# Bismarrck/tensoralloy

Measured on AMD Instinct MI355X. Metric: atom-steps/sec (energy+forces), 4000-atom Ni rcut=6.5 A, higher is better.
Workload: dtype f64

## Files before the change

### tensoralloy_amd/csrc/ta_api.hip

```cpp
#include <hip/hip_runtime.h>

#include <algorithm>
#include <chrono>
#include <climits>
#include <cmath>
#include <cstdio>
#include <cstdlib>
#include <cstring>
#include <stdexcept>
#include <string>
#include <vector>

#include "ta_device.h"
#include "ta_internal.h"
#include "ta_md.h"
#include "ta_neb.h"
#include "ta_relax.h"

namespace ta {
size_t mlp_scratch_doubles(const MlpDev &mlp);
void launch_mlp_impl(const MlpDev &mlp, int activation, int ndim, const int32_t *atoms, int n_atoms,
                     const DeviceBatch &b, const Options &opt, double *scratch, hipStream_t s,
                     MlpLaunchInfo *info = nullptr);
size_t mlp_all_scratch_doubles(const MlpDev *mlps_host, int nel, const int32_t *elem_start);
// ... 716 lines not shown
      if (h->nl_zero.ptr != before || h->nl_zero_atoms != (int64_t)N || h->nl_zero_bins != n_bins) h->nl_zero_clean = false;
      h->nl_zero_atoms = (int64_t)N;
      h->nl_zero_bins = n_bins;
    }
    h->nl_rev_done = false;
    for (int attempt = 0; attempt < 2 && !h->nl_sorted; ++attempt) {
      const size_t capacity = std::min(std::min(h->pair_i.cap, h->pair_j.cap), h->pair_shift.cap / 3);
      h->pair_rev.ensure(capacity);
      const size_t guess = (hp.n_atoms == (int64_t)N && hp.n_pairs > 0) ? (size_t)hp.n_pairs + (size_t)hp.n_pairs / 4 + 4096
                                                                         : capacity;
      const size_t rev_cover = std::min(std::min(capacity, guess), (size_t)INT32_MAX);
      NlWork w = nl_work(h);
      nl_build((int)N, n_bins, nel, h->r_list, h->db.pos, h->db.species, h->db.frame_of_atom, h->d_grids, w,
               h->nl_zero.ptr, h->nl_zero_clean, (long long)std::min<size_t>(capacity, (size_t)INT32_MAX), h->pair_start.ptr,
               kernel_writes_host ? starts : nullptr, h->pair_i.ptr, h->pair_j.ptr, h->pair_shift.ptr,
               h->pair_rev.ptr, (long long)rev_cover, s);
      HIP_CHECK(hipGetLastError());
      h->nl_zero_clean = false;
      if (!kernel_writes_host)
        staged_copy(reinterpret_cast<double *>(starts), reinterpret_cast<const double *>(h->pair_start.ptr),
                    (N + 2) / 2, true, h->opt, s);
      staged_copy(reinterpret_cast<double *>(stats), reinterpret_cast<const double *>(h->nl_zero.ptr), 8, true, h->opt, s);
      wait_stream(s, h->opt);
      h->nl_zero_clean = N > 0;
      if (si[3] != 0) break;
      if (stats[4] > (unsigned long long)INT32_MAX) throw std::runtime_error("batch too large for 32-bit pair indices");
      if (stats[4] <= capacity) {
        h->nl_sorted = true;
        h->nl_rev_done = stats[4] <= rev_cover;
        if (h->nl_rev_done && si[6] != 0)
          throw std::runtime_error("neighbour list is not symmetric (reverse pair missing)");
      } else {
        h->pair_i.ensure((size_t)stats[4]);
        h->pair_j.ensure((size_t)stats[4]);
        h->pair_shift.ensure(3 * (size_t)stats[4]);
      }
    }
    if (h->nl_sorted) h->nl_stats_ptr = h->nl_zero.ptr;
  }
  if (!h->nl_sorted) {
    h->nl_bin_count.ensure((size_t)n_bins + 1);
    h->nl_bin_cursor.ensure((size_t)n_bins + 1);
    h->nl_counts.ensure(N * (nel + 1) + 1);
    h->nl_stats.ensure(8);
    NlWork w = nl_work(h);
    nl_count((int)N, n_bins, nel, h->r_list, h->db.pos, h->db.species, h->db.frame_of_atom, h->d_grids, w,
             h->pair_start.ptr, s);
    HIP_CHECK(hipGetLastError());
    HIP_CHECK(hipMemcpyAsync(stats, h->nl_stats.ptr, 8 * sizeof(unsigned long long), hipMemcpyDeviceToHost, s));
    HIP_CHECK(hipMemcpyAsync(starts, h->pair_start.ptr, (N + 1) * sizeof(int32_t), hipMemcpyDeviceToHost, s));
    HIP_CHECK(hipStreamSynchronize(s));
    if (stats[4] > (unsigned long long)INT32_MAX || si[4] < 0 || (unsigned long long)si[4] != stats[4])
      throw std::runtime_error("batch too large for 32-bit pair indices");
    h->nl_stats_ptr = h->nl_stats.ptr;
  }
  hp.n_atoms = (int64_t)N;
  hp.n_pairs = (int64_t)stats[4];
  hp.n_triples = (int64_t)stats[0];
  hp.nnl_max = si[2];
  hp.pair_start.assign(starts, starts + N + 1);
  hp.seg_start.clear();
  hp.pair_i.clear();
  hp.pair_j.clear();
  hp.pair_shift.clear();
  hp.pair_rev.clear();
  h->pairs_on_device = true;
}

void fill_pairs_on_device(ta_context *h) {
  using namespace ta;
  if (h->nl_sorted) {
    nl_reverse_sorted(h->hp.n_pairs, h->n_elements, h->db.species, h->seg_start.ptr, h->pair_i.ptr,
                      h->pair_j.ptr, h->pair_shift.ptr, h->pair_rev.ptr, h->nl_stats_ptr, h->stream);
  } else {
    NlWork w = nl_work(h);
    nl_fill((int)h->hp.n_atoms, h->hp.n_pairs, h->n_elements, h->r_list, h->db.pos, h->db.species,
            h->db.frame_of_atom, h->d_grids, w, h->pair_i.ptr, h->pair_j.ptr, h->pair_shift.ptr,
            h->pair_rev.ptr, h->stream);
  }
  HIP_CHECK(hipGetLastError());
}

#ifdef TA_PHASE_STAMPS
static void dump_stamps(ta_context *h) {
  const std::string &path = h->opt.phase_stamps_out;
  if (path.empty() || !h->db.stamps || h->db.n_blk <= 0) return;
  const size_t n = (size_t)2 * h->db.n_blk * ta::kStampSlots;
  std::vector<unsigned long long> v(n);
  (void)hipStreamSynchronize(h->stream);
  (void)hipMemcpy(v.data(), h->db.stamps, n * sizeof(unsigned long long), hipMemcpyDeviceToHost);
  FILE *fp = std::fopen(path.c_str(), "w");
  if (!fp) return;
  for (int k = 0; k < 2; ++k)
    for (int b = 0; b < h->db.n_blk; ++b) {
      std::fprintf(fp, "%d %d", k, b);
      for (int q = 0; q < ta::kStampSlots; ++q)
        std::fprintf(fp, " %llu", v[((size_t)k * h->db.n_blk + b) * ta::kStampSlots + q]);
      std::fprintf(fp, "\n");
    }
  std::fclose(fp);
}
#endif

void launch_head(ta_context *h, const ta::DeviceBatch &db, hipStream_t s) {
  if (h->td)
    ta::launch_td_all(h->td_dev, h->td_nets, h->n_elements, h->td_K, h->td_act, h->activation,
                      h->td_sommerfeld ? 1 : 0, h->sf.ndim, db, h->opt.mlp_da_global, h->td_T.ptr, h->td_u.ptr, h->td_s.ptr,
                      h->mlp_scratch.ptr, s, &h->last_mlp_launch);
  else
    ta::launch_mlp_all(h->mlp_dev, h->mlp, h->n_elements, h->activation, h->sf.ndim, db, h->opt, h->mlp_scratch.ptr,
                       s, &h->last_mlp_launch);
}

void forward_v2_launches(ta_context *h, bool tri) {
  using namespace ta;
  bool unread = tri && h->db.job_word_own && h->db.job_count_own && h->db.job_count;
  for (const ChunkPlan &cp : h->chunks_v2) unread = unread && v2_backward_takes_triangles(h->sf, cp.ch, cp.ng, cp.nz);
  bool geometry = true;
  size_t left = h->chunks_v2.size();
  for (const ChunkPlan &cp : h->chunks_v2) {
    --left;
    launch_g4_forward_v2(h->sf, cp.ch, cp.ng, cp.nz, geometry, left == 0, unread, h->db, h->opt, h->stream);
    geometry = false;
  }
  h->full_jobs_valid = !unread;
}

void compute_impl(ta_context *h, uint32_t want, bool timed, double *slot_ms) {
  using namespace ta;
#ifdef TA_PHASE_STAMPS
  if (h->db.n_blk > 0) {
    h->stamp_buf.ensure((size_t)2 * h->db.n_blk * ta::kStampSlots + 8);
    h->db.stamps = h->stamp_buf.ptr;
    (void)hipMemsetAsync(h->db.stamps, 0, (size_t)2 * h->db.n_blk * ta::kStampSlots * sizeof(unsigned long long),
                         h->stream);
  }
#endif
  h->db.rec4 = nullptr;
  h->db.own_sums = 0;
  const DeviceBatch &db = h->db;
  hipStream_t s = h->stream;
  const bool need_forces = (want & (TA_WANT_FORCES | TA_WANT_VIRIAL)) != 0;
  auto begin = [&](int slot) {
    if (timed) HIP_CHECK(hipEventRecord(h->ev[2 * slot], s));
  };
  auto end = [&](int slot) {
    if (timed) HIP_CHECK(hipEventRecord(h->ev[2 * slot + 1], s));
  };
  bool used[TA_N_KERNEL_SLOTS] = {false};

  const bool has_mlp = h->kind == TA_MODEL_SF_MLP || h->kind == TA_MODEL_GRAP_MLP;
  if ((want & TA_WANT_REUSE_DESCRIPTORS) && has_mlp && h->descriptors_valid && !need_forces) {
    begin(TA_K_MLP);
    launch_head(h, db, s);
    end(TA_K_MLP);
    used[TA_K_MLP] = true;
  } else if (h->kind == TA_MODEL_SF_MLP) {
    h->db.rec4 = (h->sf.angular && h->use_v2 && !h->opt.full_records) ? h->db.rec : nullptr;
    if (!h->use_v2) {
      begin(TA_K_PAIR_GEOMETRY);
      launch_pair_geometry(h->sf, db, s);
      end(TA_K_PAIR_GEOMETRY);
      used[TA_K_PAIR_GEOMETRY] = true;
    }
    h->sf.ang_scale = h->use_v2 ? 1.0 : 0.5;
    const bool tri_cells = (h->relax_cell_on || h->md_baro_on) ? h->tri_cells_wide_ok : h->tri_cells_ok;
    const bool tri = h->use_v2 && h->triangles && tri_cells && h->n_elements == 1 && need_forces;
    h->db.job_word_own = (tri && h->db.job_count) ? h->job_word_own.ptr : nullptr;
    h->db.job_count_own = (tri && h->db.job_count) ? h->job_count_own.ptr : nullptr;
    h->last_bwd_variant = 0;
    const bool reduce_in_forward = h->sf.angular && h->use_v2;
    if (h->sf.angular) {
      begin(TA_K_G4_FORWARD);
      if (h->use_v2)
        forward_v2_launches(h, tri);
      else
        for (const ChunkPlan &cp : h->chunks) launch_g4_forward(h->sf, cp.ch, cp.nb, cp.ng, cp.nz, db, s);
      end(TA_K_G4_FORWARD);
      used[TA_K_G4_FORWARD] = true;
    }
    if (!reduce_in_forward) {
      begin(TA_K_DESCRIPTOR_REDUCE);
      launch_descriptor_reduce(h->sf, db, s);
      end(TA_K_DESCRIPTOR_REDUCE);
      used[TA_K_DESCRIPTOR_REDUCE] = true;
    }
    begin(TA_K_MLP);
    launch_head(h, db, s);
    end(TA_K_MLP);
    used[TA_K_MLP] = true;
    if (need_forces) {
      begin(TA_K_BACKWARD);
      if (h->sf.angular) {
        bool first = true;
        if (h->use_v2)
          for (const ChunkPlan &cp : h->chunks_v2) {
            h->last_bwd_variant |= launch_backward_v2(h->sf, cp.ch, cp.ng, cp.nz, first, tri, db, h->opt, s);
            first = false;
          }
        else
          for (const ChunkPlan &cp : h->chunks) {
            launch_backward(h->sf, cp.ch, cp.nb, cp.ng, cp.nz, first, false, db, s);
            first = false;
          }
      } else {
        AngChunk dummy;
        std::memset(&dummy, 0, sizeof(dummy));
        launch_backward(h->sf, dummy, 1, 1, 1, true, true, db, s);
      }
      end(TA_K_BACKWARD);
      used[TA_K_BACKWARD] = true;
      begin(TA_K_FORCE_GATHER);
      launch_force_gather(h->sf, db, h->opt.gather_w, s);
      end(TA_K_FORCE_GATHER);
      used[TA_K_FORCE_GATHER] = true;
    }
  } else if (h->kind == TA_MODEL_GRAP_MLP) {
    const bool net_exact = ta::grap_uses_filter_net(h->grap) && !ta::grap_filter_table_knots(h->grap);
// ... 3056 lines not shown
```

### tensoralloy_amd/csrc/ta_mlp.hip

```cpp
#include <hip/hip_runtime.h>

#include <algorithm>
#include <cstdlib>
#include <map>
#include <mutex>
#include <stdexcept>

#include "ta_device.h"
#include "ta_mlp_tile.h"

namespace ta {
namespace {

constexpr int kMlpThreads = 256;

template <int THREADS>
__global__ __launch_bounds__(THREADS) void mlp_kernel(MlpDev mlp, int act, int ndim,
                                                          const int32_t *atoms, int n_atoms,
                                                          const double *G, double *dEdG,
                                                          double *eatom, double *scratch, int stride) {
  extern __shared__ double lds[];
  double *buf0 = lds, *buf1 = lds + kMlpRows * stride;
  const int a0 = blockIdx.x * kMlpRows;
  const int nrows = min(kMlpRows, n_atoms - a0);
  double *da = scratch ? scratch + (size_t)blockIdx.x * mlp.n_layers * kMlpRows * stride
                       : lds + 2 * kMlpRows * stride;
  for (int idx = threadIdx.x; idx < kMlpRows * ndim; idx += THREADS) {
    const int row = idx / ndim, k = idx - row * ndim;
    buf0[row * stride + k] = row < nrows ? G[(size_t)atoms[a0 + row] * ndim + k] : 0.0;
  }
  __syncthreads();
  mlp_tile<16>(
      mlp, act, ndim, nrows, buf0, buf1, stride, da,
      [&](int row, double y) { eatom[atoms[a0 + row]] = y; },
      [&](int row, int k, double d) { dEdG[(size_t)atoms[a0 + row] * ndim + k] = d; });
}

struct MlpTiles {
  int32_t tile_start[kMaxElements + 1];
  int32_t elem_start[kMaxElements + 1];
  int nel;
};

template <int THREADS>
__global__ __launch_bounds__(THREADS) void mlp_all_kernel(const MlpDev *__restrict__ mlps, MlpTiles tiles, int act,
                                                              int ndim, const int32_t *atoms,
                                                              const double *G, double *dEdG,
                                                              double *eatom, double *scratch,
                                                              int stride, int tile_doubles) {
  extern __shared__ double lds[];
  double *buf0 = lds, *buf1 = lds + kMlpRows * stride;
  int e = 0;
  while (e + 1 < tiles.nel && (int)blockIdx.x >= tiles.tile_start[e + 1]) ++e;
  const MlpDev &mlp = mlps[e];
  const int32_t *el_atoms = atoms + tiles.elem_start[e];
  const int n_atoms = tiles.elem_start[e + 1] - tiles.elem_start[e];
  const int a0 = ((int)blockIdx.x - tiles.tile_start[e]) * kMlpRows;
  const int nrows = min(kMlpRows, n_atoms - a0);
  double *da = scratch ? scratch + (size_t)blockIdx.x * tile_doubles : lds + 2 * kMlpRows * stride;
  for (int idx = threadIdx.x; idx < kMlpRows * ndim; idx += THREADS) {
    const int row = idx / ndim, k = idx - row * ndim;
    buf0[row * stride + k] = row < nrows ? G[(size_t)el_atoms[a0 + row] * ndim + k] : 0.0;
  }
  __syncthreads();
  mlp_tile<16>(
      mlp, act, ndim, nrows, buf0, buf1, stride, da,
      [&](int row, double y) { eatom[el_atoms[a0 + row]] = y; },
      [&](int row, int k, double d) { dEdG[(size_t)el_atoms[a0 + row] * ndim + k] = d; });
}

constexpr int kWaveNT = 4;
constexpr int kWaveThreads = 512;
constexpr int kWaveMaxHidden = 3;

constexpr int kWaveStride = 80;
__host__ __device__ inline int wave_stride(int x) { return (x % 32 == 0) ? x + 16 : x; }

struct WaveLds {
  const double *w[kWaveMaxHidden], *wt[kWaveMaxHidden], *b[kWaveMaxHidden];
  int swt0;
  const double *wout;
  double bout;
};

__host__ __device__ inline size_t wave_lds_doubles(const MlpDev &mlp, int lh) {
  size_t n = 0;
  for (int l = 0; l < lh; ++l) {
    const MlpLayerDev &ly = mlp.layer[l];
    n += (size_t)ly.kp * kWaveStride + (size_t)ly.np * (l == 0 ? wave_stride(ly.kp) : kWaveStride) + ly.np;
  }
  return n + mlp.layer[lh].kp;
}

__device__ __forceinline__ void wave_copy_rows(double *dst, int stride, const double *__restrict__ src, int rows,
                                               int cols) {
  const int n = rows * cols;
  for (int base = 0; base < n; base += 8 * kWaveThreads) {
    double v[8];
#pragma unroll
    for (int u = 0; u < 8; ++u) {
      const int idx = base + u * kWaveThreads + (int)threadIdx.x;
      v[u] = idx < n ? src[idx] : 0.0;
    }
#pragma unroll
    for (int u = 0; u < 8; ++u) {
      const int idx = base + u * kWaveThreads + (int)threadIdx.x;
      if (idx < n) {
        const int row = idx / cols;
        dst[row * stride + (idx - row * cols)] = v[u];
      }
    }
  }
}

template <int LH>
__device__ __forceinline__ void wave_stage(const MlpDev &mlp, double *lds, WaveLds &L) {
  double *p = lds;
#pragma unroll
// ... 148 lines not shown
      if (t < ntp) {
#pragma unroll
        for (int r = 0; r < 4; ++r) dh[l - 1][t][r] *= acc[t][r];
      }
  }
  {
    const MlpLayerDev &ly = mlp.layer[0];
    const int nt0 = ly.np / 16, swt = L.swt0;
    for (int j0 = 0; j0 < ndim; j0 += 16) {
      mlp_f64x4 acc = {0.0, 0.0, 0.0, 0.0};
      const double *wcol = L.wt[0] + kq * swt + j0 + m;
#pragma unroll
      for (int nt = 0; nt < kWaveNT; ++nt) {
        if (nt >= nt0) continue;
        double a[4];
#pragma unroll
        for (int r = 0; r < 4; ++r) a[r] = wcol[(16 * nt + 4 * r) * swt];
#pragma unroll
        for (int r = 0; r < 4; ++r) acc = __builtin_amdgcn_mfma_f64_16x16x4f64(a[r], dh[0][nt][r], acc, 0, 0, 0);
      }
#pragma unroll
      for (int r = 0; r < 4; ++r) {
        const int j = j0 + kq + 4 * r;
        if (valid && j < ndim) {
          double d = acc[r];
          if (mlp.xlo) {
            const double den = mlp.xhi[j] - mlp.xlo[j];
            d = (den != 0.0) ? -d / den : 0.0;
          }
          dEdG[(size_t)atom * ndim + j] = d;
        }
      }
    }
  }
}

template <int LH>
__global__ __launch_bounds__(kWaveThreads) void mlp_wave_kernel(MlpDev mlp, int act, int ndim, const int32_t *atoms,
                                                                int n_atoms, const double *G, double *dEdG,
                                                                double *eatom) {
  extern __shared__ double lds[];
  WaveLds L;
  wave_stage<LH>(mlp, lds, L);
  __syncthreads();
  const int ntiles = (n_atoms + kMlpRows - 1) / kMlpRows, nw = kWaveThreads / 64;
  for (int tile = (int)blockIdx.x * nw + (int)(threadIdx.x >> 6); tile < ntiles; tile += (int)gridDim.x * nw)
    mlp_wave_tile<LH>(mlp, L, act, ndim, atoms, n_atoms, tile * kMlpRows, G, dEdG, eatom);
}

template <int LH>
__global__ __launch_bounds__(kWaveThreads) void mlp_wave_all_kernel(const MlpDev *__restrict__ mlps, MlpTiles tiles,
                                                                    int act, int ndim, const int32_t *atoms,
                                                                    const double *G, double *dEdG, double *eatom) {
  extern __shared__ double lds[];
  const int e = blockIdx.y;
  const int n_atoms = tiles.elem_start[e + 1] - tiles.elem_start[e];
  const int ntiles = (n_atoms + kMlpRows - 1) / kMlpRows, nw = kWaveThreads / 64;
  if ((int)blockIdx.x * nw >= ntiles) return;
  const MlpDev &mlp = mlps[e];
  WaveLds L;
  wave_stage<LH>(mlp, lds, L);
  __syncthreads();
  for (int tile = (int)blockIdx.x * nw + (int)(threadIdx.x >> 6); tile < ntiles; tile += (int)gridDim.x * nw)
    mlp_wave_tile<LH>(mlp, L, act, ndim, atoms + tiles.elem_start[e], n_atoms, tile * kMlpRows, G, dEdG, eatom);
}

}

size_t mlp_scratch_doubles(const MlpDev &mlp) {
  return (size_t)mlp.n_layers * kMlpRows * mlp_stride(mlp);
}

constexpr size_t kWaveLdsLimit = 150 * 1024;

int mlp_quad_shape(const MlpDev &mlp, int n_tiles, const Options &opt);
int mlp_quad_tiles(const MlpDev &mlp);

template <int NT>
struct QuadLds {
  double h[2][16 * NT * kMlpRows];
  double ypart[NT][kMlpRows];
};

template <int NT>
__device__ __forceinline__ void quad_fetch(double (&w)[4 * NT], const double *wcol, size_t stride, int n_tiles) {
#pragma unroll
  for (int t = 0; t < NT; ++t)
#pragma unroll
    for (int r = 0; r < 4; ++r) w[4 * t + r] = t < n_tiles ? wcol[(size_t)(16 * t + 4 * r) * stride] : 0.0;
}
template <int NT>
__device__ __forceinline__ mlp_f64x4 quad_gemm(const double (&w)[4 * NT], const double *bin, int n_tiles,
                                               mlp_f64x4 acc) {
#pragma unroll
  for (int t = 0; t < NT; ++t)
    if (t < n_tiles) {
      double bq[4];
#pragma unroll
      for (int r = 0; r < 4; ++r) bq[r] = bin[(16 * t + 4 * r) * kMlpRows];
#pragma unroll
      for (int r = 0; r < 4; ++r) acc = __builtin_amdgcn_mfma_f64_16x16x4f64(w[4 * t + r], bq[r], acc, 0, 0, 0);
    }
  return acc;
}

template <int LH, int NT>
__device__ __forceinline__ void mlp_quad_body(const MlpDev &mlp, QuadLds<NT> &L, int act, int ndim,
                                              const int32_t *atoms, int n_atoms, int a0,
                                              const double *__restrict__ G, double *__restrict__ dEdG,
                                              double *__restrict__ eatom) {
  const int lane = threadIdx.x & 63, nt = threadIdx.x >> 6, m = lane & 15, kq = lane >> 4;
  const bool valid = a0 + m < n_atoms;
  const int atom = atoms[valid ? a0 + m : a0];
  mlp_f64x4 dh[LH];
  int cur = 0;
  {
    const MlpLayerDev &ly = mlp.layer[0];
    if (nt < ly.np / 16) {
      mlp_f64x4 acc;
#pragma unroll
      for (int r = 0; r < 4; ++r) acc[r] = ly.b[16 * nt + kq + 4 * r];
      const double *g = G + (size_t)atom * ndim;
      for (int k0 = 0; k0 < ndim; k0 += 4) {
        const int k = k0 + kq;
        double x = 0.0;
        if (k < ndim) {
          x = g[k];
          if (mlp.xlo) {
            const double den = mlp.xhi[k] - mlp.xlo[k];
            x = (den != 0.0) ? (mlp.xhi[k] - x) / den : 0.0;
          }
        }
        acc = __builtin_amdgcn_mfma_f64_16x16x4f64(ly.w[(size_t)k * ly.np + 16 * nt + m], x, acc, 0, 0, 0);
      }
#pragma unroll
      for (int r = 0; r < 4; ++r) {
        double hv, dv;
        activation_fn(act, acc[r], hv, dv);
        dh[0][r] = dv;
        L.h[cur][(16 * nt + kq + 4 * r) * kMlpRows + m] = hv;
      }
    }
  }
  double wnext[4 * NT];
  mlp_f64x4 bnext = {0.0, 0.0, 0.0, 0.0};
  __syncthreads();
  if (LH > 1) {
    const MlpLayerDev &nx = mlp.layer[1];
    const int tile = nt < nx.np / 16 ? nt : 0;
    quad_fetch<NT>(wnext, nx.w + (size_t)kq * nx.np + 16 * tile + m, nx.np, nx.kp / 16);
#pragma unroll
    for (int r = 0; r < 4; ++r) bnext[r] = nx.b[16 * tile + kq + 4 * r];
  } else {
    const MlpLayerDev &l0 = mlp.layer[0];
    quad_fetch<NT>(wnext, l0.wt + (size_t)kq * l0.kp + (16 * nt < ndim ? 16 * nt : 0) + m, l0.kp, l0.np / 16);
  }
#pragma unroll
  for (int l = 1; l < LH; ++l) {
    const MlpLayerDev &ly = mlp.layer[l];
    mlp_f64x4 acc = bnext;
    if (nt < ly.np / 16) acc = quad_gemm<NT>(wnext, L.h[cur] + kq * kMlpRows + m, ly.kp / 16, acc);
    if (nt < ly.np / 16) {
#pragma unroll
      for (int r = 0; r < 4; ++r) {
        double hv, dv;
        activation_fn(act, acc[r], hv, dv);
        dh[l][r] = dv;
        L.h[cur ^ 1][(16 * nt + kq + 4 * r) * kMlpRows + m] = hv;
      }
    }
    cur ^= 1;
    __syncthreads();
    if (l + 1 < LH) {
      const MlpLayerDev &nx = mlp.layer[l + 1];
      const int tile = nt < nx.np / 16 ? nt : 0;
      quad_fetch<NT>(wnext, nx.w + (size_t)kq * nx.np + 16 * tile + m, nx.np, nx.kp / 16);
#pragma unroll
      for (int r = 0; r < 4; ++r) bnext[r] = nx.b[16 * tile + kq + 4 * r];
    } else {
      const int tile = nt < ly.kp / 16 ? nt : 0;
      quad_fetch<NT>(wnext, ly.wt + (size_t)kq * ly.kp + 16 * tile + m, ly.kp, ly.np / 16);
    }
  }
  {
    const MlpLayerDev &lo = mlp.layer[LH];
    double y = 0.0;
    if (nt < lo.kp / 16) {
#pragma unroll
      for (int r = 0; r < 4; ++r) {
        const int k = 16 * nt + kq + 4 * r;
        const double wo = lo.w[(size_t)k * lo.np];
        y = fma(L.h[cur][k * kMlpRows + m], wo, y);
        L.h[cur ^ 1][k * kMlpRows + m] = dh[LH - 1][r] * wo;
      }
    }
    y += __shfl_xor(y, 16);
    y += __shfl_xor(y, 32);
    if (kq == 0) L.ypart[nt][m] = y;
    cur ^= 1;
    __syncthreads();
    if (nt == 0 && kq == 0 && valid) {
      double y4[NT / 4];
#pragma unroll
      for (int q = 0; q < NT / 4; ++q)
        y4[q] = (L.ypart[4 * q][m] + L.ypart[4 * q + 1][m]) + (L.ypart[4 * q + 2][m] + L.ypart[4 * q + 3][m]);
      double ys = y4[0];
#pragma unroll
      for (int q = 1; q < NT / 4; ++q) ys += y4[q];
      eatom[atom] = ys + lo.b[0];
    }
  }
#pragma unroll
  for (int l = LH - 1; l >= 1; --l) {
    const MlpLayerDev &ly = mlp.layer[l];
    mlp_f64x4 acc = {0.0, 0.0, 0.0, 0.0};
    if (nt < ly.kp / 16) acc = quad_gemm<NT>(wnext, L.h[cur] + kq * kMlpRows + m, ly.np / 16, acc);
    if (nt < ly.kp / 16) {
#pragma unroll
      for (int r = 0; r < 4; ++r) L.h[cur ^ 1][(16 * nt + kq + 4 * r) * kMlpRows + m] = acc[r] * dh[l - 1][r];
    }
    cur ^= 1;
    __syncthreads();
    {
      const MlpLayerDev &nx = mlp.layer[l - 1];
      const int col = l > 1 ? (nt < nx.kp / 16 ? 16 * nt : 0) : (16 * nt < ndim ? 16 * nt : 0);
      quad_fetch<NT>(wnext, nx.wt + (size_t)kq * nx.kp + col + m, nx.kp, nx.np / 16);
    }
  }
  {
    const MlpLayerDev &ly = mlp.layer[0];
    for (int j0 = 16 * nt; j0 < ndim; j0 += 16 * NT) {
      mlp_f64x4 acc = {0.0, 0.0, 0.0, 0.0};
      if (j0 != 16 * nt) quad_fetch<NT>(wnext, ly.wt + (size_t)kq * ly.kp + j0 + m, ly.kp, ly.np / 16);
      acc = quad_gemm<NT>(wnext, L.h[cur] + kq * kMlpRows + m, ly.np / 16, acc);
#pragma unroll
      for (int r = 0; r < 4; ++r) {
        const int j = j0 + kq + 4 * r;
        if (valid && j < ndim) {
          double d = acc[r];
          if (mlp.xlo) {
            const double den = mlp.xhi[j] - mlp.xlo[j];
            d = (den != 0.0) ? -d / den : 0.0;
          }
          dEdG[(size_t)atom * ndim + j] = d;
        }
      }
    }
  }
}


template <int LH, int NT>
__global__ __launch_bounds__(64 * NT) void mlp_quad_kernel(MlpDev mlp, int act, int ndim, const int32_t *atoms,
                                                           int n_atoms, const double *__restrict__ G,
                                                           double *__restrict__ dEdG, double *__restrict__ eatom) {
  __shared__ QuadLds<NT> L;
  mlp_quad_body<LH, NT>(mlp, L, act, ndim, atoms, n_atoms, (int)blockIdx.x * kMlpRows, G, dEdG, eatom);
}

template <int LH, int NT>
__global__ __launch_bounds__(64 * NT) void mlp_quad_all_kernel(const MlpDev *__restrict__ mlps, MlpTiles tiles,
                                                               int act, int ndim, const int32_t *atoms,
                                                               const double *__restrict__ G,
                                                               double *__restrict__ dEdG,
                                                               double *__restrict__ eatom) {
  __shared__ QuadLds<NT> L;
  int e = 0;
  while (e + 1 < tiles.nel && (int)blockIdx.x >= tiles.tile_start[e + 1]) ++e;
  mlp_quad_body<LH, NT>(mlps[e], L, act, ndim, atoms + tiles.elem_start[e],
                        tiles.elem_start[e + 1] - tiles.elem_start[e],
                        ((int)blockIdx.x - tiles.tile_start[e]) * kMlpRows, G, dEdG, eatom);
}

constexpr int kWaveMinTiles = 1024;

int mlp_wave_shape(const MlpDev &mlp, int n_tiles, const Options &opt) {
  const int lh = mlp.n_layers - 1;
  if (lh < 1 || lh > kWaveMaxHidden || opt.mlp_tile_kernel) return 0;
  if (n_tiles < kWaveMinTiles && !opt.mlp_wave_kernel) return 0;
  for (int l = 0; l < lh; ++l) {
    const MlpLayerDev &ly = mlp.layer[l];
    if (ly.np > 16 * kWaveNT || ly.res || !ly.act) return 0;
    if (l > 0 && ly.kp != mlp.layer[l - 1].np) return 0;
  }
  const MlpLayerDev &lo = mlp.layer[lh];
  if (lo.n != 1 || lo.act || lo.res || lo.kp != mlp.layer[lh - 1].np) return 0;
  if (wave_lds_doubles(mlp, lh) * sizeof(double) > kWaveLdsLimit) return 0;
  return lh;
}

constexpr int kQuadMinTiles = 257;
constexpr int kQuadMaxNT = 8;

int mlp_quad_tiles(const MlpDev &mlp) {
  const int lh = mlp.n_layers - 1;
  if (lh < 1 || lh > kWaveMaxHidden) return 0;
  int widest = 0;
  for (int l = 0; l < lh; ++l) {
    const MlpLayerDev &ly = mlp.layer[l];
    if (ly.np > 16 * kQuadMaxNT || ly.res || !ly.act) return 0;
    if (l > 0 && ly.kp != mlp.layer[l - 1].np) return 0;
    widest = std::max(widest, ly.np);
  }
  const MlpLayerDev &lo = mlp.layer[lh];
  if (lo.n != 1 || lo.act || lo.res || lo.kp != mlp.layer[lh - 1].np) return 0;
  return widest <= 16 * kWaveNT ? kWaveNT : kQuadMaxNT;
}

int mlp_quad_shape(const MlpDev &mlp, int n_tiles, const Options &opt) {
  if (opt.mlp_tile_kernel || opt.mlp_wave_kernel) return 0;
  const int nt = mlp_quad_tiles(mlp);
  if (!nt) return 0;
  if (opt.mlp_quad_kernel) return mlp.n_layers - 1;
  if (nt == kWaveNT && (n_tiles >= kWaveMinTiles || n_tiles < kQuadMinTiles)) return 0;
  if (nt == kQuadMaxNT && n_tiles >= 4 * kWaveMinTiles) return 0;
  return mlp.n_layers - 1;
}

template <typename K>
void allow_lds(K kernel, size_t bytes) {
  if (bytes <= 64 * 1024) return;
  static std::mutex mu;
  static std::map<std::pair<const void *, int>, size_t> allowed;
  int dev = 0;
  (void)hipGetDevice(&dev);
  const auto key = std::make_pair(reinterpret_cast<const void *>(kernel), dev);
  std::lock_guard<std::mutex> lock(mu);
  auto it = allowed.find(key);
  if (it != allowed.end() && it->second >= bytes) return;
  if (hipFuncSetAttribute(key.first, hipFuncAttributeMaxDynamicSharedMemorySize, (int)kWaveLdsLimit) != hipSuccess)
    throw std::runtime_error("hipFuncSetAttribute(MaxDynamicSharedMemorySize) failed");
  allowed[key] = kWaveLdsLimit;
}

void launch_mlp_impl(const MlpDev &mlp, int activation, int ndim, const int32_t *atoms, int n_atoms,
                     const DeviceBatch &b, const Options &opt, double *scratch, hipStream_t s, MlpLaunchInfo *info) {
  if (n_atoms == 0) return;
  auto note = [&](int family, int threads, int lh, int nt, unsigned gx, unsigned gy, size_t lds, int da) {
    if (info) *info = MlpLaunchInfo{family, threads, lh, nt, (int)gx, (int)gy, (long long)lds, da};
  };
  if (const int lh = mlp_quad_shape(mlp, (n_atoms + kMlpRows - 1) / kMlpRows, opt)) {
    const unsigned qblocks = (unsigned)((n_atoms + kMlpRows - 1) / kMlpRows);
    const int nt = mlp_quad_tiles(mlp);
    note(TA_MLP_QUAD, 64 * nt, lh, nt, qblocks, 1, 0, TA_MLP_DA_REGISTERS);
#define TA_QUAD(LH, NT)                                                                                       \
  hipLaunchKernelGGL((mlp_quad_kernel<LH, NT>), dim3(qblocks), dim3(64 * NT), 0, s, mlp, activation, ndim, atoms, \
                     n_atoms, b.G, b.dEdG, b.eatom)
    if (nt == kWaveNT) {
      if (lh == 1) TA_QUAD(1, 4);
      else if (lh == 2) TA_QUAD(2, 4);
      else TA_QUAD(3, 4);
    } else {
      if (lh == 1) TA_QUAD(1, 8);
      else if (lh == 2) TA_QUAD(2, 8);
      else TA_QUAD(3, 8);
    }
#undef TA_QUAD
    return;
  }
  if (const int lh = mlp_wave_shape(mlp, (n_atoms + kMlpRows - 1) / kMlpRows, opt)) {
    const int ntiles = (n_atoms + kMlpRows - 1) / kMlpRows, nw = kWaveThreads / 64;
    const unsigned wblocks = (unsigned)std::min((ntiles + nw - 1) / nw, 256);
    const size_t lds = wave_lds_doubles(mlp, lh) * sizeof(double);
    note(TA_MLP_WAVE, kWaveThreads, lh, 0, wblocks, 1, lds, TA_MLP_DA_REGISTERS);
    auto go = [&](auto kernel) {
      allow_lds(kernel, lds);
      hipLaunchKernelGGL(kernel, dim3(wblocks), dim3(kWaveThreads), lds, s, mlp, activation, ndim, atoms, n_atoms,
                         b.G, b.dEdG, b.eatom);
    };
    if (lh == 1) go(mlp_wave_kernel<1>);
    else if (lh == 2) go(mlp_wave_kernel<2>);
    else go(mlp_wave_kernel<3>);
    return;
  }
  const int stride = mlp_stride(mlp);
  size_t lds = 2 * (size_t)kMlpRows * stride * sizeof(double);
  const unsigned blocks = (unsigned)((n_atoms + kMlpRows - 1) / kMlpRows);
  const size_t lds_da = (size_t)mlp.n_layers * kMlpRows * stride * sizeof(double);
  int da = TA_MLP_DA_GLOBAL;
  if (lds + lds_da <= 64 * 1024 && !opt.mlp_da_global) {
    lds += lds_da;
    scratch = nullptr;
    da = TA_MLP_DA_LDS;
  }
  note(TA_MLP_TILE, mlp.max_np >= 128 ? 512 : kMlpThreads, 0, 0, blocks, 1, lds, da);
  if (mlp.max_np >= 128)
    hipLaunchKernelGGL(mlp_kernel<512>, dim3(blocks), dim3(512), lds, s, mlp, activation, ndim, atoms,
                       n_atoms, b.G, b.dEdG, b.eatom, scratch, stride);
  else
    hipLaunchKernelGGL(mlp_kernel<kMlpThreads>, dim3(blocks), dim3(kMlpThreads), lds, s, mlp, activation,
                       ndim, atoms, n_atoms, b.G, b.dEdG, b.eatom, scratch, stride);
}

size_t mlp_all_scratch_doubles(const MlpDev *mlps_host, int nel, const int32_t *elem_start) {
  int stride = 0, layers = 0;
  size_t tiles = 0;
  for (int e = 0; e < nel; ++e) {
    stride = std::max(stride, mlp_stride(mlps_host[e]));
    layers = std::max(layers, mlps_host[e].n_layers);
    tiles += (size_t)(elem_start[e + 1] - elem_start[e] + kMlpRows - 1) / kMlpRows;
  }
  return tiles * layers * kMlpRows * stride;
}

void launch_mlp_all(const MlpDev *mlps_dev, const MlpDev *mlps_host, int nel, int activation, int ndim,
                    const DeviceBatch &b, const Options &opt, double *scratch, hipStream_t s, MlpLaunchInfo *info) {
  if (info) *info = MlpLaunchInfo{};
  auto note = [&](int family, int threads, int lh, int nt, unsigned gx, unsigned gy, size_t lds, int da) {
    if (info) *info = MlpLaunchInfo{family, threads, lh, nt, (int)gx, (int)gy, (long long)lds, da};
  };
  if (nel == 1) {
    launch_mlp_impl(mlps_host[0], activation, ndim, b.elem_atoms, b.elem_start[1] - b.elem_start[0], b,
                    opt, scratch, s, info);
    return;
  }
  MlpTiles t;
  t.nel = nel;
  int stride = 0, layers = 0, blocks = 0, width = 0;
  for (int e = 0; e < nel; ++e) {
    width = std::max(width, mlps_host[e].max_np);
    stride = std::max(stride, mlp_stride(mlps_host[e]));
    layers = std::max(layers, mlps_host[e].n_layers);
    t.tile_start[e] = blocks;
    t.elem_start[e] = b.elem_start[e];
    blocks += (b.elem_start[e + 1] - b.elem_start[e] + kMlpRows - 1) / kMlpRows;
  }
  t.tile_start[nel] = blocks;
  t.elem_start[nel] = b.elem_start[nel];
  for (int e = nel + 1; e <= kMaxElements; ++e) t.tile_start[e] = t.elem_start[e] = 0;
  if (blocks == 0) return;
  {
    int qlh = mlp_quad_shape(mlps_host[0], blocks, opt), qnt = mlp_quad_tiles(mlps_host[0]);
    for (int e = 1; e < nel; ++e)
      if (mlp_quad_shape(mlps_host[e], blocks, opt) != qlh || mlp_quad_tiles(mlps_host[e]) != qnt) qlh = 0;
    if (qlh) {
      note(TA_MLP_QUAD_ALL, 64 * qnt, qlh, qnt, (unsigned)blocks, 1, 0, TA_MLP_DA_REGISTERS);
#define TA_QUAD_ALL(LH, NT)                                                                                \
  hipLaunchKernelGGL((mlp_quad_all_kernel<LH, NT>), dim3((unsigned)blocks), dim3(64 * NT), 0, s, mlps_dev, t, \
                     activation, ndim, b.elem_atoms, b.G, b.dEdG, b.eatom)
      if (qnt == kWaveNT) {
        if (qlh == 1) TA_QUAD_ALL(1, 4);
        else if (qlh == 2) TA_QUAD_ALL(2, 4);
        else TA_QUAD_ALL(3, 4);
      } else {
        if (qlh == 1) TA_QUAD_ALL(1, 8);
        else if (qlh == 2) TA_QUAD_ALL(2, 8);
        else TA_QUAD_ALL(3, 8);
      }
#undef TA_QUAD_ALL
      return;
    }
  }
  int lh = mlp_wave_shape(mlps_host[0], blocks, opt);
  size_t wlds = 0;
  int max_tiles = 0;
  for (int e = 0; e < nel; ++e) {
    if (mlp_wave_shape(mlps_host[e], blocks, opt) != lh) lh = 0;
    if (lh) wlds = std::max(wlds, wave_lds_doubles(mlps_host[e], lh) * sizeof(double));
    max_tiles = std::max(max_tiles, (b.elem_start[e + 1] - b.elem_start[e] + kMlpRows - 1) / kMlpRows);
  }
  if (lh) {
    const int nw = kWaveThreads / 64;
    const unsigned wblocks = (unsigned)std::min((max_tiles + nw - 1) / nw, std::max(256 / nel, 1));
    note(TA_MLP_WAVE_ALL, kWaveThreads, lh, 0, wblocks, (unsigned)nel, wlds, TA_MLP_DA_REGISTERS);
    auto go = [&](auto kernel) {
      allow_lds(kernel, wlds);
      hipLaunchKernelGGL(kernel, dim3(wblocks, (unsigned)nel), dim3(kWaveThreads), wlds, s, mlps_dev, t, activation,
                         ndim, b.elem_atoms, b.G, b.dEdG, b.eatom);
    };
    if (lh == 1) go(mlp_wave_all_kernel<1>);
    else if (lh == 2) go(mlp_wave_all_kernel<2>);
    else go(mlp_wave_all_kernel<3>);
    return;
  }
// ... 21 lines not shown
```

### tensoralloy_amd/csrc/ta_mlp_tile.h

```cpp
#pragma once
#include <hip/hip_runtime.h>

#include "ta_device.h"
#include "ta_math.h"

namespace ta {

typedef double mlp_f64x4 __attribute__((ext_vector_type(4)));
constexpr int kMlpRows = 16;

template <int PF, typename Emit>
__device__ __forceinline__ void mlp_tile_gemm(const double *X, int xstride, const double *W,
                                              int wstride, int kp, int np, const double *bias,
                                              int lane, int wave, int nwaves, Emit emit) {
  const int m = lane & 15, kq = lane >> 4;
  for (int nt = wave; nt < np / 16; nt += nwaves) {
    const int col = 16 * nt + m;
    const double b0 = bias ? bias[col] : 0.0;
    mlp_f64x4 acc = {b0, b0, b0, b0};
    const int nk = kp / 4;
    int kk0 = 0;
    if constexpr (PF > 4) {
      for (; kk0 + PF <= nk; kk0 += PF) {
        double w[PF];
#pragma unroll
        for (int j = 0; j < PF; ++j) w[j] = W[(size_t)(4 * (kk0 + j) + kq) * wstride + col];
#pragma unroll
        for (int j = 0; j < PF; ++j)
          acc = __builtin_amdgcn_mfma_f64_16x16x4f64(X[m * xstride + 4 * (kk0 + j) + kq], w[j], acc, 0, 0, 0);
      }
    }
    for (; kk0 < nk; kk0 += 4) {
      double a[4], w[4];
#pragma unroll
      for (int j = 0; j < 4; ++j) {
        w[j] = W[(size_t)(4 * (kk0 + j) + kq) * wstride + col];
        a[j] = X[m * xstride + 4 * (kk0 + j) + kq];
      }
#pragma unroll
      for (int j = 0; j < 4; ++j) acc = __builtin_amdgcn_mfma_f64_16x16x4f64(a[j], w[j], acc, 0, 0, 0);
    }
#pragma unroll
    for (int r = 0; r < 4; ++r) emit(kq + 4 * r, col, acc[r]);
  }
}

template <int PF = 4, typename EmitE, typename EmitG>
__device__ __forceinline__ void mlp_tile(const MlpDev &mlp, int act, int ndim, int nrows,
                                         double *buf0, double *buf1, int stride, double *da,
                                         EmitE emit_energy, EmitG emit_grad) {
  const int tid = threadIdx.x, nthreads = blockDim.x;
  const int lane = tid & 63, wave = tid >> 6, nwaves = nthreads >> 6;
  const int L = mlp.n_layers;

  const int kp0 = mlp.layer[0].kp;
  for (int idx = tid; idx < kMlpRows * kp0; idx += nthreads) {
    const int row = idx / kp0, k = idx - row * kp0;
    double x = 0.0;
    if (row < nrows && k < ndim) {
      x = buf0[row * stride + k];
      if (mlp.xlo) {
        const double den = mlp.xhi[k] - mlp.xlo[k];
        x = (den != 0.0) ? (mlp.xhi[k] - x) / den : 0.0;
      }
    }
    buf1[row * stride + k] = x;
  }
  __syncthreads();

  double *cur = buf1, *nxt = buf0;
  for (int l = 0; l < L; ++l) {
    const MlpLayerDev ly = mlp.layer[l];
    double *dal = da + (size_t)l * kMlpRows * stride;
    mlp_tile_gemm<PF>(cur, stride, ly.w, ly.np, ly.kp, ly.np, ly.b, lane, wave, nwaves,
                  [&](int row, int col, double z) {
                    double h = 0.0, dh = 0.0;
                    if (row < nrows) {
                      h = z;
                      dh = 1.0;
                      if (ly.act) activation_fn(act, z, h, dh);
                      if (ly.res) h += cur[row * stride + col];
                    }
                    nxt[row * stride + col] = h;
                    dal[row * stride + col] = dh;
                  });
    __syncthreads();
    double *t = cur;
    cur = nxt;
    nxt = t;
  }
  if (tid < nrows) emit_energy(tid, cur[tid * stride]);
  __syncthreads();

  const int npL = mlp.layer[L - 1].np;
  for (int idx = tid; idx < kMlpRows * npL; idx += nthreads) {
    const int row = idx / npL, col = idx - row * npL;
    cur[row * stride + col] = (col == 0) ? 1.0 : 0.0;
  }
  __syncthreads();
  for (int l = L - 1; l >= 0; --l) {
    const MlpLayerDev ly = mlp.layer[l];
    const double *dal = da + (size_t)l * kMlpRows * stride;
    if (ly.res) {
      for (int idx = tid; idx < kMlpRows * ly.np; idx += nthreads) {
        const int row = idx / ly.np, col = idx - row * ly.np;
        nxt[row * stride + col] = cur[row * stride + col];
      }
    }
    for (int idx = tid; idx < kMlpRows * ly.np; idx += nthreads) {
      const int row = idx / ly.np, col = idx - row * ly.np;
      cur[row * stride + col] *= dal[row * stride + col];
    }
    __syncthreads();
    const bool res = ly.res != 0;
    double *dst = nxt;
    mlp_tile_gemm<PF>(cur, stride, ly.wt, ly.kp, ly.np, ly.kp, nullptr, lane, wave, nwaves,
                  [&](int row, int col, double z) {
                    const double skip = res ? dst[row * stride + col] : 0.0;
                    dst[row * stride + col] = z + skip;
                  });
    __syncthreads();
    double *t = cur;
    cur = nxt;
    nxt = t;
  }
  for (int idx = tid; idx < kMlpRows * ndim; idx += nthreads) {
    const int row = idx / ndim, k = idx - row * ndim;
    if (row >= nrows) continue;
    double d = cur[row * stride + k];
    if (mlp.xlo) {
      const double den = mlp.xhi[k] - mlp.xlo[k];
      d = (den != 0.0) ? -d / den : 0.0;
    }
    emit_grad(row, k, d);
  }
  __syncthreads();
}

inline int mlp_stride(const MlpDev &mlp) {
  const int w = mlp.max_np > mlp.max_kp ? mlp.max_np : mlp.max_kp;
  return w + 2;
}

}
```

Measured before the change: 39.27 million.

## Prefetch next-layer MLP weights earlier in quad kernel and batch first-layer loads

```diff
diff --git a/tensoralloy_amd/csrc/ta_api.hip b/tensoralloy_amd/csrc/ta_api.hip
--- a/tensoralloy_amd/csrc/ta_api.hip
+++ b/tensoralloy_amd/csrc/ta_api.hip
@@ -822,10 +822,11 @@
 }
 
 #ifdef TA_PHASE_STAMPS
+static size_t stamp_mlp_rows(const ta_context *h) { return (size_t)(h->db.n_atoms + 15) / 16; }
 static void dump_stamps(ta_context *h) {
   const std::string &path = h->opt.phase_stamps_out;
   if (path.empty() || !h->db.stamps || h->db.n_blk <= 0) return;
-  const size_t n = (size_t)2 * h->db.n_blk * ta::kStampSlots;
+  const size_t n = ((size_t)2 * h->db.n_blk + stamp_mlp_rows(h)) * ta::kStampSlots;
   std::vector<unsigned long long> v(n);
   (void)hipStreamSynchronize(h->stream);
   (void)hipMemcpy(v.data(), h->db.stamps, n * sizeof(unsigned long long), hipMemcpyDeviceToHost);
@@ -838,6 +839,12 @@
         std::fprintf(fp, " %llu", v[((size_t)k * h->db.n_blk + b) * ta::kStampSlots + q]);
       std::fprintf(fp, "\n");
     }
+  for (size_t b = 0; b < stamp_mlp_rows(h); ++b) {
+    std::fprintf(fp, "2 %zu", b);
+    for (int q = 0; q < ta::kStampSlots; ++q)
+      std::fprintf(fp, " %llu", v[((size_t)2 * h->db.n_blk + b) * ta::kStampSlots + q]);
+    std::fprintf(fp, "\n");
+  }
   std::fclose(fp);
 }
 #endif
@@ -870,10 +877,10 @@
   using namespace ta;
 #ifdef TA_PHASE_STAMPS
   if (h->db.n_blk > 0) {
-    h->stamp_buf.ensure((size_t)2 * h->db.n_blk * ta::kStampSlots + 8);
+    const size_t n = ((size_t)2 * h->db.n_blk + stamp_mlp_rows(h)) * ta::kStampSlots;
+    h->stamp_buf.ensure(n + 8);
     h->db.stamps = h->stamp_buf.ptr;
-    (void)hipMemsetAsync(h->db.stamps, 0, (size_t)2 * h->db.n_blk * ta::kStampSlots * sizeof(unsigned long long),
-                         h->stream);
+    (void)hipMemsetAsync(h->db.stamps, 0, n * sizeof(unsigned long long), h->stream);
   }
 #endif
   h->db.rec4 = nullptr;
diff --git a/tensoralloy_amd/csrc/ta_mlp.hip b/tensoralloy_amd/csrc/ta_mlp.hip
--- a/tensoralloy_amd/csrc/ta_mlp.hip
+++ b/tensoralloy_amd/csrc/ta_mlp.hip
@@ -14,11 +14,26 @@
 
 constexpr int kMlpThreads = 256;
 
+#ifdef TA_PHASE_STAMPS
+#define TA_MLP_STAMP_PARAM , unsigned long long *stamps
+#define TA_MLP_STAMP_PASS(b) , ((b).stamps ? (b).stamps + (size_t)2 * (b).n_blk * kStampSlots : nullptr)
+#define TA_MLP_STAMP_TILE , mlp_stamps_
+#define TA_MLP_STAMP_KERNEL_ENTRY()                                                                         \
+  unsigned long long *mlp_stamps_ = stamps ? stamps + (size_t)blockIdx.x * kStampSlots : nullptr;          \
+  TA_MLP_STAMP(0)
+#else
+#define TA_MLP_STAMP_PARAM
+#define TA_MLP_STAMP_PASS(b)
+#define TA_MLP_STAMP_TILE
+#define TA_MLP_STAMP_KERNEL_ENTRY() do {} while (0)
+#endif
+
 template <int THREADS>
 __global__ __launch_bounds__(THREADS) void mlp_kernel(MlpDev mlp, int act, int ndim,
                                                           const int32_t *atoms, int n_atoms,
                                                           const double *G, double *dEdG,
-                                                          double *eatom, double *scratch, int stride) {
+                                                          double *eatom, double *scratch, int stride TA_MLP_STAMP_PARAM) {
+  TA_MLP_STAMP_KERNEL_ENTRY();
   extern __shared__ double lds[];
   double *buf0 = lds, *buf1 = lds + kMlpRows * stride;
   const int a0 = blockIdx.x * kMlpRows;
@@ -33,7 +48,7 @@
   mlp_tile<16>(
       mlp, act, ndim, nrows, buf0, buf1, stride, da,
       [&](int row, double y) { eatom[atoms[a0 + row]] = y; },
-      [&](int row, int k, double d) { dEdG[(size_t)atoms[a0 + row] * ndim + k] = d; });
+      [&](int row, int k, double d) { dEdG[(size_t)atoms[a0 + row] * ndim + k] = d; } TA_MLP_STAMP_TILE);
 }
 
 struct MlpTiles {
@@ -348,6 +363,7 @@
   double ypart[NT][kMlpRows];
 };
 
+__device__ __forceinline__ void quad_settled() { __builtin_amdgcn_s_waitcnt(0x0F70); }
 template <int NT>
 __device__ __forceinline__ void quad_fetch(double (&w)[4 * NT], const double *wcol, size_t stride, int n_tiles) {
 #pragma unroll
@@ -380,25 +396,66 @@
   const int atom = atoms[valid ? a0 + m : a0];
   mlp_f64x4 dh[LH];
   int cur = 0;
+  double wnext[4 * NT];
+  mlp_f64x4 bnext = {0.0, 0.0, 0.0, 0.0};
+  double wout[4];
+  auto fetch_behind = [&](int l) {
+    quad_settled();
+    if (l + 1 < LH) {
+      const MlpLayerDev &nx = mlp.layer[l + 1];
+      const int tile = nt < nx.np / 16 ? nt : 0;
+      quad_fetch<NT>(wnext, nx.w + (size_t)kq * nx.np + 16 * tile + m, nx.np, nx.kp / 16);
+#pragma unroll
+      for (int r = 0; r < 4; ++r) bnext[r] = nx.b[16 * tile + kq + 4 * r];
+    } else {
+      const MlpLayerDev &ly = mlp.layer[l], &lo = mlp.layer[LH];
+      const int col = l == 0 ? (16 * nt < ndim ? 16 * nt : 0) : (nt < ly.kp / 16 ? 16 * nt : 0);
+      quad_fetch<NT>(wnext, ly.wt + (size_t)kq * ly.kp + col + m, ly.kp, ly.np / 16);
+#pragma unroll
+      for (int r = 0; r < 4; ++r)
+        wout[r] = nt < lo.kp / 16 ? lo.w[(size_t)(16 * nt + kq + 4 * r) * lo.np] : 0.0;
+    }
+  };
   {
     const MlpLayerDev &ly = mlp.layer[0];
-    if (nt < ly.np / 16) {
-      mlp_f64x4 acc;
+    const bool mine = nt < ly.np / 16;
+    mlp_f64x4 acc = {0.0, 0.0, 0.0, 0.0};
+    if (mine) {
 #pragma unroll
       for (int r = 0; r < 4; ++r) acc[r] = ly.b[16 * nt + kq + 4 * r];
       const double *g = G + (size_t)atom * ndim;
-      for (int k0 = 0; k0 < ndim; k0 += 4) {
-        const int k = k0 + kq;
-        double x = 0.0;
-        if (k < ndim) {
-          x = g[k];
-          if (mlp.xlo) {
-            const double den = mlp.xhi[k] - mlp.xlo[k];
-            x = (den != 0.0) ? (mlp.xhi[k] - x) / den : 0.0;
+      constexpr int kQuadK0 = 8;
+      for (int c0 = 0; c0 < ndim; c0 += 4 * kQuadK0) {
+        double x[kQuadK0], w[kQuadK0], hi[kQuadK0], lo[kQuadK0];
+#pragma unroll
+        for (int j = 0; j < kQuadK0; ++j) {
+          const int k = c0 + 4 * j + kq;
+          x[j] = w[j] = hi[j] = lo[j] = 0.0;
+          if (c0 + 4 * j < ndim) {
+            w[j] = ly.w[(size_t)k * ly.np + 16 * nt + m];
+            if (k < ndim) {
+              x[j] = g[k];
+              if (mlp.xlo) {
+                hi[j] = mlp.xhi[k];
+                lo[j] = mlp.xlo[k];
+              }
+            }
           }
         }
-        acc = __builtin_amdgcn_mfma_f64_16x16x4f64(ly.w[(size_t)k * ly.np + 16 * nt + m], x, acc, 0, 0, 0);
-      }
+#pragma unroll
+        for (int j = 0; j < kQuadK0; ++j) {
+          if (c0 + 4 * j >= ndim) break;
+          double xs = x[j];
+          if (mlp.xlo && c0 + 4 * j + kq < ndim) {
+            const double den = hi[j] - lo[j];
+            xs = (den != 0.0) ? (hi[j] - xs) / den : 0.0;
+          }
+          acc = __builtin_amdgcn_mfma_f64_16x16x4f64(w[j], xs, acc, 0, 0, 0);
+        }
+      }
+    }
+    fetch_behind(0);
+    if (mine) {
 #pragma unroll
       for (int r = 0; r < 4; ++r) {
         double hv, dv;
@@ -408,24 +465,13 @@
       }
     }
   }
-  double wnext[4 * NT];
-  mlp_f64x4 bnext = {0.0, 0.0, 0.0, 0.0};
   __syncthreads();
-  if (LH > 1) {
-    const MlpLayerDev &nx = mlp.layer[1];
-    const int tile = nt < nx.np / 16 ? nt : 0;
-    quad_fetch<NT>(wnext, nx.w + (size_t)kq * nx.np + 16 * tile + m, nx.np, nx.kp / 16);
-#pragma unroll
-    for (int r = 0; r < 4; ++r) bnext[r] = nx.b[16 * tile + kq + 4 * r];
-  } else {
-    const MlpLayerDev &l0 = mlp.layer[0];
-    quad_fetch<NT>(wnext, l0.wt + (size_t)kq * l0.kp + (16 * nt < ndim ? 16 * nt : 0) + m, l0.kp, l0.np / 16);
-  }
 #pragma unroll
   for (int l = 1; l < LH; ++l) {
     const MlpLayerDev &ly = mlp.layer[l];
     mlp_f64x4 acc = bnext;
     if (nt < ly.np / 16) acc = quad_gemm<NT>(wnext, L.h[cur] + kq * kMlpRows + m, ly.kp / 16, acc);
+    fetch_behind(l);
     if (nt < ly.np / 16) {
 #pragma unroll
       for (int r = 0; r < 4; ++r) {
@@ -437,16 +483,6 @@
     }
     cur ^= 1;
     __syncthreads();
-    if (l + 1 < LH) {
-      const MlpLayerDev &nx = mlp.layer[l + 1];
-      const int tile = nt < nx.np / 16 ? nt : 0;
-      quad_fetch<NT>(wnext, nx.w + (size_t)kq * nx.np + 16 * tile + m, nx.np, nx.kp / 16);
-#pragma unroll
-      for (int r = 0; r < 4; ++r) bnext[r] = nx.b[16 * tile + kq + 4 * r];
-    } else {
-      const int tile = nt < ly.kp / 16 ? nt : 0;
-      quad_fetch<NT>(wnext, ly.wt + (size_t)kq * ly.kp + 16 * tile + m, ly.kp, ly.np / 16);
-    }
   }
   {
     const MlpLayerDev &lo = mlp.layer[LH];
@@ -455,7 +491,7 @@
 #pragma unroll
       for (int r = 0; r < 4; ++r) {
         const int k = 16 * nt + kq + 4 * r;
-        const double wo = lo.w[(size_t)k * lo.np];
+        const double wo = wout[r];
         y = fma(L.h[cur][k * kMlpRows + m], wo, y);
         L.h[cur ^ 1][k * kMlpRows + m] = dh[LH - 1][r] * wo;
       }
@@ -481,17 +517,18 @@
     const MlpLayerDev &ly = mlp.layer[l];
     mlp_f64x4 acc = {0.0, 0.0, 0.0, 0.0};
     if (nt < ly.kp / 16) acc = quad_gemm<NT>(wnext, L.h[cur] + kq * kMlpRows + m, ly.np / 16, acc);
-    if (nt < ly.kp / 16) {
-#pragma unroll
-      for (int r = 0; r < 4; ++r) L.h[cur ^ 1][(16 * nt + kq + 4 * r) * kMlpRows + m] = acc[r] * dh[l - 1][r];
-    }
-    cur ^= 1;
-    __syncthreads();
     {
       const MlpLayerDev &nx = mlp.layer[l - 1];
       const int col = l > 1 ? (nt < nx.kp / 16 ? 16 * nt : 0) : (16 * nt < ndim ? 16 * nt : 0);
+      quad_settled();
       quad_fetch<NT>(wnext, nx.wt + (size_t)kq * nx.kp + col + m, nx.kp, nx.np / 16);
     }
+    if (nt < ly.kp / 16) {
+#pragma unroll
+      for (int r = 0; r < 4; ++r) L.h[cur ^ 1][(16 * nt + kq + 4 * r) * kMlpRows + m] = acc[r] * dh[l - 1][r];
+    }
+    cur ^= 1;
+    __syncthreads();
   }
   {
     const MlpLayerDev &ly = mlp.layer[0];
@@ -652,10 +689,10 @@
   note(TA_MLP_TILE, mlp.max_np >= 128 ? 512 : kMlpThreads, 0, 0, blocks, 1, lds, da);
   if (mlp.max_np >= 128)
     hipLaunchKernelGGL(mlp_kernel<512>, dim3(blocks), dim3(512), lds, s, mlp, activation, ndim, atoms,
-                       n_atoms, b.G, b.dEdG, b.eatom, scratch, stride);
+                       n_atoms, b.G, b.dEdG, b.eatom, scratch, stride TA_MLP_STAMP_PASS(b));
   else
     hipLaunchKernelGGL(mlp_kernel<kMlpThreads>, dim3(blocks), dim3(kMlpThreads), lds, s, mlp, activation,
-                       ndim, atoms, n_atoms, b.G, b.dEdG, b.eatom, scratch, stride);
+                       ndim, atoms, n_atoms, b.G, b.dEdG, b.eatom, scratch, stride TA_MLP_STAMP_PASS(b));
 }
 
 size_t mlp_all_scratch_doubles(const MlpDev *mlps_host, int nel, const int32_t *elem_start) {
diff --git a/tensoralloy_amd/csrc/ta_mlp_tile.h b/tensoralloy_amd/csrc/ta_mlp_tile.h
--- a/tensoralloy_amd/csrc/ta_mlp_tile.h
+++ b/tensoralloy_amd/csrc/ta_mlp_tile.h
@@ -8,6 +8,17 @@
 
 typedef double mlp_f64x4 __attribute__((ext_vector_type(4)));
 constexpr int kMlpRows = 16;
+
+#ifdef TA_PHASE_STAMPS
+#define TA_MLP_STAMP_ARG , unsigned long long *mlp_stamps_ = nullptr
+#define TA_MLP_STAMP(k)                                                                    \
+  do {                                                                                     \
+    if (mlp_stamps_ && threadIdx.x == 0 && (k) < kStampSlots) mlp_stamps_[k] = __builtin_amdgcn_s_memrealtime(); \
+  } while (0)
+#else
+#define TA_MLP_STAMP_ARG
+#define TA_MLP_STAMP(k) do {} while (0)
+#endif
 
 template <int PF, typename Emit>
 __device__ __forceinline__ void mlp_tile_gemm(const double *X, int xstride, const double *W,
@@ -48,7 +59,7 @@
 template <int PF = 4, typename EmitE, typename EmitG>
 __device__ __forceinline__ void mlp_tile(const MlpDev &mlp, int act, int ndim, int nrows,
                                          double *buf0, double *buf1, int stride, double *da,
-                                         EmitE emit_energy, EmitG emit_grad) {
+                                         EmitE emit_energy, EmitG emit_grad TA_MLP_STAMP_ARG) {
   const int tid = threadIdx.x, nthreads = blockDim.x;
   const int lane = tid & 63, wave = tid >> 6, nwaves = nthreads >> 6;
   const int L = mlp.n_layers;
@@ -67,6 +78,7 @@
     buf1[row * stride + k] = x;
   }
   __syncthreads();
+  TA_MLP_STAMP(1);
 
   double *cur = buf1, *nxt = buf0;
   for (int l = 0; l < L; ++l) {
@@ -85,11 +97,13 @@
                     dal[row * stride + col] = dh;
                   });
     __syncthreads();
+    TA_MLP_STAMP(2 + l);
     double *t = cur;
     cur = nxt;
     nxt = t;
   }
   if (tid < nrows) emit_energy(tid, cur[tid * stride]);
+  TA_MLP_STAMP(2 + L);
   __syncthreads();
 
   const int npL = mlp.layer[L - 1].np;
@@ -120,6 +134,7 @@
                     dst[row * stride + col] = z + skip;
                   });
     __syncthreads();
+    TA_MLP_STAMP(3 + L + (L - 1 - l));
     double *t = cur;
     cur = nxt;
     nxt = t;
@@ -135,6 +150,7 @@
     emit_grad(row, k, d);
   }
   __syncthreads();
+  TA_MLP_STAMP(3 + 2 * L);
 }
 
 inline int mlp_stride(const MlpDev &mlp) {
```

After: 38.50 million. 0.98x the previous value.
